# fishaudio/fish-diffusion

Hardware: NVIDIA H100
Metric: mel_frames_per_sec_100step_ddpm (higher is better)
Workload: dtype f32 (3x fp16 split-product wgmma, fp32 accumulate)

## Files before the change

fish_diffusion_b200/csrc/fd_common.cuh:

```cuda
#pragma once
#include <cuda_runtime.h>
#include <cuda_fp16.h>
#include <cuda_bf16.h>
#include <stdint.h>

#define FD_F16 0
#define FD_BF16 1
#define FD_SINGLE 0x10

#define FD_MAX_SEG 16

#define FD_EPI_LINEAR 0
#define FD_EPI_GATE 1
#define FD_EPI_RES_SKIP 2
#define FD_EPI_MAG 3
#define FD_EPI_GATE_BWD 4

#define FD_ACT_NONE 0
#define FD_ACT_RELU 1
#define FD_ACT_LRELU 2
#define FD_ACT_GELU 3

struct FdSeg {
  int src;
// ... 73 lines not shown

__device__ __forceinline__ void fd_split(float v, int prec, uint16_t& hi, uint16_t& lo) {
  if (prec == FD_F16) {
    v = fminf(fmaxf(v, -65504.f), 65504.f);
    __half h = __float2half_rn(v);
    __half l = __float2half_rn(v - __half2float(h));
    hi = __half_as_ushort(h);
    lo = __half_as_ushort(l);
  } else {
    __nv_bfloat16 h = __float2bfloat16_rn(v);
    __nv_bfloat16 l = __float2bfloat16_rn(v - __bfloat162float(h));
    hi = __bfloat16_as_ushort(h);
    lo = __bfloat16_as_ushort(l);
  }
}

__device__ __forceinline__ float fd_h2f(uint16_t u, int prec) {
  if (prec == FD_F16) return __half2float(__ushort_as_half(u));
  return __uint_as_float(((uint32_t)u) << 16);
}

__device__ __forceinline__ float fd_combine(uint16_t hi, uint16_t lo, int prec) {
  return fd_h2f(hi, prec) + fd_h2f(lo, prec);
}

__device__ __forceinline__ void fd_combine2(uint32_t hi2, uint32_t lo2, int prec, float& a, float& b) {
  if (prec == FD_F16) {
    const float2 h = __half22float2(*reinterpret_cast<const __half2*>(&hi2));
    const float2 l = __half22float2(*reinterpret_cast<const __half2*>(&lo2));
    a = h.x + l.x; b = h.y + l.y;
  } else {
    a = __uint_as_float(hi2 << 16) + __uint_as_float(lo2 << 16);
    b = __uint_as_float(hi2 & 0xffff0000u) + __uint_as_float(lo2 & 0xffff0000u);
  }
}

__device__ __forceinline__ float fd_act(float w, float slope) { return fmaf(slope, fminf(w, 0.f), fmaxf(w, 0.f)); }

__device__ __forceinline__ float fd_gelu(float x) { return 0.5f * x * (1.f + erff(x * 0.70710678118654752440f)); }

__device__ __forceinline__ float fd_sigmoid(float x) { return __fdividef(1.f, 1.f + __expf(-x)); }
__device__ __forceinline__ float fd_tanh(float x) {
  float ax = fabsf(x);
  if (ax < 0.04f) { float x2 = x * x; return x * (1.f - x2 * (0.33333333f - 0.13333333f * x2)); }
  float e = __expf(2.f * ax);
  float r = 1.f - __fdividef(2.f, e + 1.f);
  return copysignf(r, x);
}

__device__ __forceinline__ void fd_dgate(float dz, float g, float f, float& dg, float& df) {
  const float sg = fd_sigmoid(g), th = fd_tanh(f);
  dg = dz * th * sg * (1.f - sg);
  df = dz * sg * (1.f - th * th);
}

__device__ __forceinline__ void fd_split2(float a, float b, int prec, uint32_t& hi2, uint32_t& lo2) {
  if (prec == FD_F16) {
    asm("cvt.rn.satfinite.f16x2.f32 %0, %1, %2;" : "=r"(hi2) : "f"(b), "f"(a));
    const float2 hf = __half22float2(*reinterpret_cast<const __half2*>(&hi2));
    asm("cvt.rn.satfinite.f16x2.f32 %0, %1, %2;" : "=r"(lo2) : "f"(b - hf.y), "f"(a - hf.x));
  } else {
    asm("cvt.rn.satfinite.bf16x2.f32 %0, %1, %2;" : "=r"(hi2) : "f"(b), "f"(a));
    const float ha = __uint_as_float(hi2 << 16), hb = __uint_as_float(hi2 & 0xffff0000u);
    asm("cvt.rn.satfinite.bf16x2.f32 %0, %1, %2;" : "=r"(lo2) : "f"(b - hb), "f"(a - ha));
  }
}

template <int V>
__device__ __forceinline__ void fd_store_planes(uint16_t* planes, size_t plane_elems, size_t off,
                                                const float (&y)[V], int prec) {
  uint32_t hi[V / 2], lo[V / 2];
#pragma unroll
  for (int i = 0; i < V / 2; ++i) fd_split2(y[2 * i], y[2 * i + 1], prec, hi[i], lo[i]);
  if (V == 4) {
    *reinterpret_cast<uint2*>(planes + off) = make_uint2(hi[0], hi[1]);
    *reinterpret_cast<uint2*>(planes + plane_elems + off) = make_uint2(lo[0], lo[1]);
  } else {
    *reinterpret_cast<uint4*>(planes + off) = make_uint4(hi[0], hi[1], hi[2 % (V / 2)], hi[3 % (V / 2)]);
    *reinterpret_cast<uint4*>(planes + plane_elems + off) = make_uint4(lo[0], lo[1], lo[2 % (V / 2)], lo[3 % (V / 2)]);
  }
}

template <int V>
__device__ __forceinline__ void fd_load_planes(const uint16_t* planes, size_t plane_elems, size_t off,
                                               float (&y)[V], int prec) {
  uint32_t hi[4], lo[4];
  if (V == 4) {
    const uint2 a = *reinterpret_cast<const uint2*>(planes + off);
    const uint2 b = *reinterpret_cast<const uint2*>(planes + plane_elems + off);
    hi[0] = a.x; hi[1] = a.y; lo[0] = b.x; lo[1] = b.y;
  } else {
    const uint4 a = *reinterpret_cast<const uint4*>(planes + off);
    const uint4 b = *reinterpret_cast<const uint4*>(planes + plane_elems + off);
    hi[0] = a.x; hi[1] = a.y; hi[2] = a.z; hi[3] = a.w; lo[0] = b.x; lo[1] = b.y; lo[2] = b.z; lo[3] = b.w;
  }
#pragma unroll
  for (int i = 0; i < V / 2; ++i) fd_combine2(hi[i], lo[i], prec, y[2 * i], y[2 * i + 1]);
}

__device__ __forceinline__ void fd_load_hi8(const uint16_t* planes, size_t off, float (&y)[8], int prec) {
  const uint4 a = *reinterpret_cast<const uint4*>(planes + off);
  const uint32_t w[4] = {a.x, a.y, a.z, a.w};
#pragma unroll
  for (int i = 0; i < 4; ++i) {
    y[2 * i] = fd_h2f((uint16_t)(w[i] & 0xffff), prec);
    y[2 * i + 1] = fd_h2f((uint16_t)(w[i] >> 16), prec);
  }
}

template <int V>
__device__ __forceinline__ void fd_load_f32(const float* p, float (&y)[V]) {
#pragma unroll
  for (int i = 0; i < V; i += 4) {
    float4 q = *reinterpret_cast<const float4*>(p + i);
    y[i] = q.x; y[i + 1] = q.y; y[i + 2] = q.z; y[i + 3] = q.w;
  }
}
template <int V>
__device__ __forceinline__ void fd_store_f32(float* p, const float (&y)[V]) {
#pragma unroll
  for (int i = 0; i < V; i += 4)
    *reinterpret_cast<float4*>(p + i) = make_float4(y[i], y[i + 1], y[i + 2], y[i + 3]);
}

template <typename I>
struct FdRows {
  I item;
  int t0, dt, nrows;
  __device__ __forceinline__ I row(const FdTapGemm& p, int r) const { return item + (I)min(t0 + r * dt, p.T - 1); }
};

__device__ __forceinline__ int fd_gate_col(const FdTapGemm& p, int c) {
  const int half = p.gate_tile / 2;
  return (c / half) * p.gate_tile + c % half;
}

template <int R, int V, int PREC, typename I>
__device__ __forceinline__ void fd_epi_linear(const FdTapGemm& p, const FdRows<I>& rw, int n, float (&a)[R][V],
                                              const float (&bias)[V]) {
  const int prec = PREC < 0 ? p.prec : PREC;
  const size_t plane = (size_t)p.B * p.T * p.n_total;
  I off[R];
  float pre[R][V];
#pragma unroll
  for (int r = 0; r < R; ++r) {
    off[r] = rw.row(p, r) * (I)p.n_total + (I)n;
#pragma unroll
    for (int i = 0; i < V; ++i) pre[r][i] = 0.f;
  }
  if (p.addend != nullptr) {
#pragma unroll
    for (int r = 0; r < R; ++r) {
      float v[V];
      fd_load_f32<V>(p.addend + off[r], v);
#pragma unroll
      for (int i = 0; i < V; ++i) pre[r][i] += v[i];
    }
  }
  if (p.res_f32 != nullptr) {
#pragma unroll
    for (int r = 0; r < R; ++r) {
      float v[V];
      fd_load_f32<V>(p.res_f32 + off[r], v);
#pragma unroll
      for (int i = 0; i < V; ++i) pre[r][i] += v[i];
    }
  }
  if (p.res_planes != nullptr) {
#pragma unroll
    for (int r = 0; r < R; ++r) {
      float v[V];
      fd_load_planes<V>(p.res_planes, plane, off[r], v, prec);
#pragma unroll
      for (int i = 0; i < V; ++i) pre[r][i] += p.res_scale * v[i];
    }
  }
  uint32_t masked = 0;
  if (p.row_mask != nullptr) {
#pragma unroll
    for (int r = 0; r < R; ++r)
      if (p.row_mask[rw.row(p, r)] != 0) masked |= 1u << r;
  }
#pragma unroll
  for (int r = 0; r < R; ++r)
#pragma unroll
    for (int i = 0; i < V; ++i) a[r][i] = (a[r][i] * p.acc_scale + bias[i] + pre[r][i]) * p.post_scale;
  if (p.out_f32 != nullptr && p.out_accum) {
#pragma unroll
    for (int r = 0; r < R; ++r) {
      float v[V];
      fd_load_f32<V>(p.out_f32 + off[r], v);
#pragma unroll
      for (int i = 0; i < V; ++i) a[r][i] += v[i];
    }
  }
  const float slope = p.act == FD_ACT_NONE ? 1.f : p.act == FD_ACT_RELU ? 0.f : p.act_slope;
#pragma unroll
  for (int r = 0; r < R; ++r) {
    if (r >= rw.nrows) break;
    if ((masked >> r) & 1u) {
#pragma unroll
      for (int i = 0; i < V; ++i) a[r][i] = 0.f;
    }
    if (p.out_f32 != nullptr) fd_store_f32<V>(p.out_f32 + off[r], a[r]);
    if (p.out_planes != nullptr) {
      float v[V];
      if (p.act == FD_ACT_GELU) {
#pragma unroll
        for (int i = 0; i < V; ++i) v[i] = fd_gelu(a[r][i] * p.planes_scale);
      } else {
#pragma unroll
        for (int i = 0; i < V; ++i) v[i] = fd_act(a[r][i] * p.planes_scale, slope);
      }
      fd_store_planes<V>(p.out_planes, plane, off[r], v, prec);
    }
  }
}

template <int R, int V, int PREC, typename I>
__device__ __forceinline__ void fd_epi_res_skip(const FdTapGemm& p, const FdRows<I>& rw, int n, bool is_res,
                                                const float (&a)[R][V], const float (&bias)[V]) {
  const int prec = PREC < 0 ? p.prec : PREC;
  const size_t plane = (size_t)p.B * p.T * p.C;
  const I cn = (I)(is_res ? n : n - p.C);
  I off[R];
#pragma unroll
  for (int r = 0; r < R; ++r) off[r] = rw.row(p, r) * (I)p.C + cn;
  if (is_res) {
    if (p.last_layer) return;
    float x[R][V];
#pragma unroll
    for (int r = 0; r < R; ++r) fd_load_planes<V>(p.x_planes, plane, off[r], x[r], prec);
    uint16_t* const xo = p.x_out_planes != nullptr ? p.x_out_planes : p.x_planes;
#pragma unroll
    for (int r = 0; r < R; ++r) {
      if (r >= rw.nrows) break;
#pragma unroll
      for (int i = 0; i < V; ++i) x[r][i] = (x[r][i] + (a[r][i] * p.acc_scale + bias[i])) * 0.70710678118654752440f;
      fd_store_planes<V>(xo, plane, off[r], x[r], prec);
    }
  } else {
    float sk[R][V];
    if (!p.first_layer) {
#pragma unroll
      for (int r = 0; r < R; ++r) fd_load_f32<V>(p.skip_f32 + off[r], sk[r]);
    }
#pragma unroll
    for (int r = 0; r < R; ++r) {
      if (r >= rw.nrows) break;
      float y[V];
#pragma unroll
      for (int i = 0; i < V; ++i) {
        y[i] = a[r][i] * p.acc_scale + bias[i];
        if (!p.first_layer) y[i] += sk[r][i];
      }
      if (p.last_layer) {
#pragma unroll
        for (int i = 0; i < V; ++i) y[i] *= p.skip_scale;
        fd_store_planes<V>(p.skip_planes, plane, off[r], y, prec);
      } else {
        fd_store_f32<V>(p.skip_f32 + off[r], y);
      }
    }
  }
}

template <int V>
__device__ __forceinline__ void fd_epi_gate(const FdTapGemm& p, int t, float (&g)[V], float (&f)[V], float (&z)[V],
                                            const float (&bias)[2][V], const float (&add)[2][V],
                                            const float (&lo)[2][V], const float (&hi)[2][V]) {
#pragma unroll
  for (int i = 0; i < V; ++i) {
    g[i] = g[i] * p.acc_scale + bias[0][i];
    f[i] = f[i] * p.acc_scale + bias[1][i];
  }
  if (p.addend != nullptr) {
#pragma unroll
    for (int i = 0; i < V; ++i) { g[i] += add[0][i]; f[i] += add[1][i]; }
  }
  if (t < p.dil) {
#pragma unroll
    for (int i = 0; i < V; ++i) { g[i] -= lo[0][i]; f[i] -= lo[1][i]; }
  }
  if (t + p.dil >= p.T) {
#pragma unroll
    for (int i = 0; i < V; ++i) { g[i] -= hi[0][i]; f[i] -= hi[1][i]; }
  }
#pragma unroll
  for (int i = 0; i < V; ++i) z[i] = fd_sigmoid(g[i]) * fd_tanh(f[i]);
}

template <int V>
struct FdColSums {
  float all[2][V], lo[2][V], hi[2][V];
};

template <int R, int V, int PREC, typename I>
__device__ __forceinline__ void fd_epi_gate_bwd(const FdTapGemm& p, const FdRows<I>& rw, int n, const float (&a)[R][V],
                                                FdColSums<V>& s) {
  const int prec = PREC < 0 ? p.prec : PREC;
  const int half = p.gate_tile / 2;
  const I w2 = 2 * (I)p.C, pg = (I)fd_gate_col(p, n);
  const size_t plane = (size_t)p.B * p.T * w2;
  I off[R];
  float g[R][V], f[R][V];
#pragma unroll
  for (int r = 0; r < R; ++r) {
    off[r] = rw.row(p, r) * w2 + pg;
    fd_load_planes<V>(p.y_planes, plane, off[r], g[r], prec);
    fd_load_planes<V>(p.y_planes, plane, off[r] + half, f[r], prec);
  }
  const bool sums = p.cs != nullptr || p.cs_edge != nullptr;
#pragma unroll
  for (int r = 0; r < R; ++r) {
    if (r >= rw.nrows) break;
    float dg[V], df[V];
#pragma unroll
    for (int i = 0; i < V; ++i) fd_dgate(a[r][i] * p.acc_scale, g[r][i], f[r][i], dg[i], df[i]);
    fd_store_planes<V>(p.out_planes, plane, off[r], dg, prec);
    fd_store_planes<V>(p.out_planes, plane, off[r] + half, df, prec);
    if (sums) {
      const int t = rw.t0 + r * rw.dt;
      const bool in_lo = t < p.dil, in_hi = t + p.dil >= p.T;
#pragma unroll
      for (int i = 0; i < V; ++i) {
        s.all[0][i] += dg[i]; s.all[1][i] += df[i];
        if (in_lo) { s.lo[0][i] += dg[i]; s.lo[1][i] += df[i]; }
        if (in_hi) { s.hi[0][i] += dg[i]; s.hi[1][i] += df[i]; }
      }
    }
  }
}

template <int FIRST_XOR, int V>
__device__ __forceinline__ void fd_gate_bwd_colsums(const FdTapGemm& p, FdColSums<V>& s, bool edge_lo, bool edge_hi,
                                                    bool lead, int b, int n) {
  if (p.cs == nullptr && p.cs_edge == nullptr) return;
  auto butterfly = [](float (&x)[2][V], int i) {
#pragma unroll
    for (int h = 0; h < 2; ++h)
#pragma unroll
      for (int o = FIRST_XOR; o < 32; o *= 2) x[h][i] += __shfl_xor_sync(0xffffffffu, x[h][i], o);
  };
#pragma unroll
// ... 73 lines not shown
```

fish_diffusion_b200/csrc/fd_tapgemm_simt.cu:

```cuda
#include "fd_common.cuh"

namespace {

constexpr int BM = 128;
constexpr int BK = 16;
constexpr int APITCH = BM + 4;

template <int RUN, int EPI>
__global__ void __launch_bounds__(256) fd_tapgemm_simt_kernel(const FdTapGemm p) {
  constexpr int BN = 2 * RUN;
  constexpr int TXC = RUN / 4;
  constexpr int TYC = 256 / TXC;
  constexpr int RM = BM / TYC;
  constexpr int BPITCH = BN + 4;

  __shared__ float As[BK][APITCH];
  __shared__ float Bs[BK][BPITCH];

  const int tid = threadIdx.x;
  const int tx = tid % TXC, ty = tid / TXC;
  const int tiles_t = (p.T + BM - 1) / BM;
  const int m_tile = blockIdx.x;
  const int b = m_tile / tiles_t;
  const int t0 = (m_tile % tiles_t) * BM;
// ... 51 lines not shown
#pragma unroll
          for (int i = 0; i < 8; ++i) v[i] = 0.f;
        }
#pragma unroll
        for (int i = 0; i < 8; ++i) Bs[kh * 8 + i][nl] = v[i];
      }
      __syncthreads();
#pragma unroll
      for (int k = 0; k < BK; ++k) {
        float a[RM], bv[8];
#pragma unroll
        for (int r = 0; r < RM; ++r) a[r] = As[k][ty * RM + r];
        float4 b0 = *reinterpret_cast<const float4*>(&Bs[k][tx * 4]);
        float4 b1 = *reinterpret_cast<const float4*>(&Bs[k][RUN + tx * 4]);
        bv[0] = b0.x; bv[1] = b0.y; bv[2] = b0.z; bv[3] = b0.w;
        bv[4] = b1.x; bv[5] = b1.y; bv[6] = b1.z; bv[7] = b1.w;
#pragma unroll
        for (int r = 0; r < RM; ++r)
#pragma unroll
          for (int c = 0; c < 8; ++c) acc[r][c] = fmaf(a[r], bv[c], acc[r][c]);
      }
      __syncthreads();
    }
    koff += sg.k_len;
  }

  const int tr = t0 + ty * RM, nrows = max(0, min(RM, p.T - tr));
  if constexpr (EPI == FD_EPI_GATE || EPI == FD_EPI_MAG) {
    const int zc = j * RUN + tx * 4, n_g = run0 + tx * 4, n_f = run1 + tx * 4;
    if (n_g >= p.n_total) return;
    const size_t zplane = (size_t)p.B * p.T * p.C, yplane = (size_t)p.B * p.T * p.n_total;
#pragma unroll
    for (int r = 0; r < RM; ++r) {
      if (r >= nrows) break;
      const int t = tr + r;
      float g[4] = {acc[r][0], acc[r][1], acc[r][2], acc[r][3]};
      float f[4] = {acc[r][4], acc[r][5], acc[r][6], acc[r][7]};
      if constexpr (EPI == FD_EPI_MAG) {
        fd_epi_mag<4>(p, b, t, zc, g, f);
      } else {
        const size_t row = (size_t)b * p.T + t, bo = (size_t)b * p.gbias_bstride;
        float add[2][4], bias[2][4], lo[2][4], hi[2][4], z[4];
        if (p.addend != nullptr) {
          fd_load_f32<4>(p.addend + row * p.n_total + n_g, add[0]);
          fd_load_f32<4>(p.addend + row * p.n_total + n_f, add[1]);
        }
#pragma unroll
        for (int i = 0; i < 4; ++i) {
          bias[0][i] = p.gbias_full[bo + n_g + i]; bias[1][i] = p.gbias_full[bo + n_f + i];
          lo[0][i] = p.gbias_lo[bo + n_g + i]; lo[1][i] = p.gbias_lo[bo + n_f + i];
          hi[0][i] = p.gbias_hi[bo + n_g + i]; hi[1][i] = p.gbias_hi[bo + n_f + i];
        }
        fd_epi_gate<4>(p, t, g, f, z, bias, add, lo, hi);
        if (p.y_planes != nullptr) {
          fd_store_planes<4>(p.y_planes, yplane, row * p.n_total + n_g, g, p.prec);
          fd_store_planes<4>(p.y_planes, yplane, row * p.n_total + n_f, f, p.prec);
        }
        fd_store_planes<4>(p.out_planes, zplane, row * p.C + zc, z, p.prec);
      }
    }
  } else {
#pragma unroll
    for (int h = 0; h < 2; ++h) {
      const int n = (h == 0 ? run0 : run1) + tx * 4;
      if constexpr (EPI == FD_EPI_GATE_BWD) {
        FdColSums<4> s{};
#pragma unroll
        for (int r = 0; r < RM; ++r) {
          if (r >= nrows || n >= p.n_total) break;
          float a[1][4] = {{acc[r][4 * h], acc[r][4 * h + 1], acc[r][4 * h + 2], acc[r][4 * h + 3]}};
          fd_epi_gate_bwd<1, 4, -1>(p, FdRows<size_t>{(size_t)b * p.T, tr + r, 1, 1}, n, a, s);
        }
        fd_gate_bwd_colsums<TXC>(p, s, t0 < p.dil, t0 + BM + p.dil > p.T, tid % 32 < TXC && n < p.n_total, b, n);
      } else {
        if (n >= p.n_total) continue;
#pragma unroll
        for (int r = 0; r < RM; ++r) {
          if (r >= nrows) break;
          float bias[4];
#pragma unroll
          for (int i = 0; i < 4; ++i) bias[i] = p.bias != nullptr ? p.bias[(size_t)b * p.bias_bstride + n + i] : 0.f;
          float a[1][4] = {{acc[r][4 * h], acc[r][4 * h + 1], acc[r][4 * h + 2], acc[r][4 * h + 3]}};
          const FdRows<size_t> row{(size_t)b * p.T, tr + r, 1, 1};
          if constexpr (EPI == FD_EPI_LINEAR) fd_epi_linear<1, 4, -1>(p, row, n, a, bias);
          else fd_epi_res_skip<1, 4, -1>(p, row, n, n < p.C, a, bias);
        }
      }
    }
  }
}

template <int RUN>
int launch_run(const FdTapGemm& p, cudaStream_t stream) {
  const int tiles_t = (p.T + BM - 1) / BM;
  dim3 grid(p.B * tiles_t, 1, 1), block(256);
  if (p.epi == FD_EPI_GATE) {
    grid.y = (p.n_total / 2 + RUN - 1) / RUN;
    fd_tapgemm_simt_kernel<RUN, FD_EPI_GATE><<<grid, block, 0, stream>>>(p);
  } else if (p.epi == FD_EPI_MAG) {
    grid.y = (p.n_total / 2 + RUN - 1) / RUN;
    fd_tapgemm_simt_kernel<RUN, FD_EPI_MAG><<<grid, block, 0, stream>>>(p);
  } else if (p.epi == FD_EPI_RES_SKIP) {
    grid.y = (p.n_total + 2 * RUN - 1) / (2 * RUN);
    fd_tapgemm_simt_kernel<RUN, FD_EPI_RES_SKIP><<<grid, block, 0, stream>>>(p);
  } else if (p.epi == FD_EPI_GATE_BWD) {
    grid.y = (p.n_total + 2 * RUN - 1) / (2 * RUN);
    fd_tapgemm_simt_kernel<RUN, FD_EPI_GATE_BWD><<<grid, block, 0, stream>>>(p);
  } else {
    grid.y = (p.n_total + 2 * RUN - 1) / (2 * RUN);
    fd_tapgemm_simt_kernel<RUN, FD_EPI_LINEAR><<<grid, block, 0, stream>>>(p);
  }
  FD_CHECK_CUDA(cudaGetLastError());
  return 0;
}

constexpr int WG_R = 64, WG_C = 64, WG_T = 16;

__global__ void __launch_bounds__(256) fd_wgrad_simt_kernel(const FdWgradK p, const uint16_t* row0,
                                                            const uint16_t* row1, const uint16_t* col0,
                                                            const uint16_t* col1, int prec, int single) {
  static_assert(WG_R == WG_C, "rows and columns share the staging code");
  __shared__ __align__(16) float Rs[WG_T][WG_R + 4];
  __shared__ __align__(16) float Cs[WG_T][WG_C + 4];
  const int tid = threadIdx.x;
  const int s = blockIdx.z, r0 = blockIdx.y * WG_R, c0 = blockIdx.x * WG_C;

  const bool is_col = tid >= 128;
  const int grp = tid % 8, tl = (tid % 128) / 8;
  const int i = (is_col ? c0 : r0) + grp * 8;
  const uint16_t* src = nullptr;
  int C = 0, ch = 0, shift = 0;
  if (!is_col) {
    for (int g = 0; g < p.num_row_seg; ++g)
      if (i >= p.row_start[g] && i < p.row_start[g] + p.row_width[g]) {
        src = p.row_src[g] == 0 ? row0 : row1;
        C = p.row_C[p.row_src[g]]; ch = p.row_coff[g] + (i - p.row_start[g]);
      }
  } else {
    for (int g = 0; g < p.num_col_seg; ++g)
      if (i >= p.col_start[g] && i < p.col_start[g] + p.col_width[g]) {
        src = p.col_src[g] == 0 ? col0 : col1;
        C = p.col_C[p.col_src[g]]; ch = p.col_coff[g] + (i - p.col_start[g]); shift = p.col_shift[g];
      }
  }
  const size_t plane = (size_t)p.B * p.T * C;
  float* const dst = is_col ? &Cs[tl][grp * 8] : &Rs[tl][grp * 8];

  const int tx = tid % 16, ty = tid / 16;
  float acc[4][4];
#pragma unroll
  for (int r = 0; r < 4; ++r)
#pragma unroll
    for (int c = 0; c < 4; ++c) acc[r][c] = 0.f;

  const int b_end = min(p.B, (s + 1) * p.items_per_split);
  for (int b = s * p.items_per_split; b < b_end; ++b) {
    for (int t0 = 0; t0 < p.T; t0 += WG_T) {
      const int t = t0 + tl, ts = t + shift;
      float v[8];
      if (src != nullptr && t < p.T && ts >= 0 && ts < p.T) {
        const size_t off = ((size_t)b * p.T + ts) * C + ch;
        if (single) fd_load_hi8(src, off, v, prec);
        else fd_load_planes<8>(src, plane, off, v, prec);
      } else {
#pragma unroll
        for (int k = 0; k < 8; ++k) v[k] = 0.f;
      }
      *reinterpret_cast<float4*>(dst) = make_float4(v[0], v[1], v[2], v[3]);
// ... 62 lines not shown
```

fish_diffusion_b200/csrc/fd_tapgemm_tc.cu:

```cuda
#include <cuda.h>
#include "fd_common.cuh"
#include "fd_host.h"
#include "fd_tc_ptx.cuh"

namespace {

constexpr int BLOCK_M = 128;

template <int BLOCK_N, int BLOCK_K, int EPI, int NPL>
struct Cfg {
  static constexpr bool PP = EPI == FD_EPI_GATE || EPI == FD_EPI_RES_SKIP;
  static constexpr int ROWS = PP ? 64 : BLOCK_M;
  static constexpr int A_BYTES = ROWS * BLOCK_K * 2;
  static constexpr int W_BYTES = BLOCK_N * BLOCK_K * 2;
  static constexpr int GROUP = BLOCK_K >= 64 || PP ? 1 : 64 / BLOCK_K;
  static constexpr int SUB_BYTES = NPL * (A_BYTES + W_BYTES);
  static constexpr int STAGE_BYTES = GROUP * SUB_BYTES;
  static constexpr int TX_BYTES = SUB_BYTES;
  static constexpr int SWIZZLE_BYTES = BLOCK_K * 2;
  static constexpr uint32_t SWIZZLE_MODE = swizzle_mode_for(SWIZZLE_BYTES);
  static constexpr uint32_t SBO = 8 * SWIZZLE_BYTES;
  static constexpr int BIAS_FLOATS = (EPI == FD_EPI_GATE ? 3 : 1) * BLOCK_N;
  static constexpr int BIAS_TOTAL = (PP ? 2 : 1) * BIAS_FLOATS;
  static constexpr int NUM_STAGES = fd_tc_frame_stages(STAGE_BYTES, BIAS_TOTAL);
  static constexpr int SMEM_BYTES = fd_tc_frame_bytes(NUM_STAGES, STAGE_BYTES, BIAS_TOTAL);
  static_assert(NUM_STAGES >= 2, "pipeline needs at least two stages");
  static_assert(SMEM_BYTES <= FD_TC_SMEM_BUDGET, "shared memory");
};

template <int BLOCK_N, int EPI>
__device__ __forceinline__ void stage_bias(const FdTapGemm& p, int b, int n0, float* bias_s, int i0, int step) {
  if (EPI == FD_EPI_GATE) {
    const size_t bo = (size_t)b * p.gbias_bstride + n0;
    for (int i = i0; i < BLOCK_N; i += step) {
      bias_s[i] = p.gbias_full[bo + i];
      bias_s[BLOCK_N + i] = p.gbias_lo[bo + i];
      bias_s[2 * BLOCK_N + i] = p.gbias_hi[bo + i];
    }
  } else {
    for (int i = i0; i < BLOCK_N; i += step)
      bias_s[i] = p.bias ? p.bias[(size_t)b * p.bias_bstride + n0 + i] : 0.f;
  }
}
template <int EPI>
__device__ __forceinline__ long long bias_key(const FdTapGemm& p, int b, int n0) {
  return EPI == FD_EPI_GATE ? (long long)b * p.gbias_bstride + n0 : (long long)b * p.bias_bstride + n0;
}

template <int BLOCK_N, int EPI, int PREC>
__device__ __forceinline__ void tile_epilogue(const FdTapGemm& p, const float* acc, int b, int n_tile, int rw0,
                                              const float* bias_s, uint32_t my_scratch, int lane) {
  const int n0 = n_tile * BLOCK_N;
  if constexpr (EPI == FD_EPI_GATE || EPI == FD_EPI_MAG) {
    constexpr int HALF = BLOCK_N / 2;
    const uint32_t sb = smem_u32(bias_s);
    const int r = lane >> 1, sub = lane & 1;
    const int t = rw0 + r;
    const bool valid = t < p.T;
    const bool e_lo = t < p.dil, e_hi = t + p.dil >= p.T;
    const bool edge_any = __any_sync(0xffffffffu, valid && (e_lo || e_hi));
    const size_t zplane = (size_t)p.B * p.T * p.C, zrow = ((size_t)b * p.T + t) * p.C + (size_t)n_tile * HALF;
    const size_t yplane = (size_t)p.B * p.T * p.n_total, yrow = ((size_t)b * p.T + t) * p.n_total;
#pragma unroll
    for (int c = 0; c < HALF; c += 16) {
      frag_to_scratch<16>(my_scratch, acc, c, 0, lane);
      frag_to_scratch<16>(my_scratch, acc, HALF + c, 16, lane);
      __syncwarp();
      float g[8], f[8];
      {
        const float4 g0 = scratch_ld4(my_scratch, r, 2 * sub), g1 = scratch_ld4(my_scratch, r, 2 * sub + 1);
        const float4 f0 = scratch_ld4(my_scratch, r, 4 + 2 * sub), f1 = scratch_ld4(my_scratch, r, 5 + 2 * sub);
        g[0] = g0.x; g[1] = g0.y; g[2] = g0.z; g[3] = g0.w; g[4] = g1.x; g[5] = g1.y; g[6] = g1.z; g[7] = g1.w;
        f[0] = f0.x; f[1] = f0.y; f[2] = f0.z; f[3] = f0.w; f[4] = f1.x; f[5] = f1.y; f[6] = f1.z; f[7] = f1.w;
      }
      __syncwarp();
      const int cc = c + 8 * sub;
      if (valid) {
        if (EPI == FD_EPI_MAG) {
          fd_epi_mag<8, PREC>(p, b, t, n_tile * HALF + cc, g, f);
        } else {
          float add[2][8], bias[2][8], lo[2][8], hi[2][8], z[8];
          if (p.addend != nullptr) {
#pragma unroll
            for (int h = 0; h < 2; ++h) ldcs_f32(p.addend + yrow + n0 + h * HALF + cc, add[h]);
          }
#pragma unroll
          for (int h = 0; h < 2; ++h) lds_f32(sb + 4u * (h * HALF + cc), bias[h]);
          if (edge_any) {
#pragma unroll
            for (int h = 0; h < 2; ++h)
              if (e_lo) lds_f32(sb + 4u * (BLOCK_N + h * HALF + cc), lo[h]);
#pragma unroll
            for (int h = 0; h < 2; ++h)
              if (e_hi) lds_f32(sb + 4u * (2 * BLOCK_N + h * HALF + cc), hi[h]);
          }
          fd_epi_gate<8>(p, t, g, f, z, bias, add, lo, hi);
          if (p.y_planes != nullptr) {
            const int ng = p.gate_tile == BLOCK_N ? n0 + cc : fd_gate_col(p, n_tile * HALF + cc);
            fd_store_planes<8>(p.y_planes, yplane, yrow + ng, g, PREC);
            fd_store_planes<8>(p.y_planes, yplane, yrow + ng + p.gate_tile / 2, f, PREC);
          }
          fd_store_planes<8>(p.out_planes, zplane, zrow + cc, z, PREC);
        }
      }
    }
  } else if constexpr (BLOCK_N >= 64) {
    const uint32_t bias_addr = smem_u32(bias_s);
    const int j4 = (lane & 7) * 4, rsub = lane >> 3;
    const int rbase = rw0 + rsub;
    const FdRows<uint32_t> rows{(uint32_t)b * (uint32_t)p.T, rbase, 4,
                                rbase < p.T ? min(4, (p.T - rbase + 3) / 4) : 0};
#pragma unroll
    for (int c = 0; c < BLOCK_N; c += 32) {
      const int col = c + j4;
      const int n = n0 + col;
      frag_to_scratch<32>(my_scratch, acc, c, 0, lane);
      __syncwarp();
      float a[4][4];
#pragma unroll
      for (int r = 0; r < 4; ++r) {
        const float4 x = scratch_ld4(my_scratch, 4 * r + rsub, lane & 7);
        a[r][0] = x.x; a[r][1] = x.y; a[r][2] = x.z; a[r][3] = x.w;
      }
      __syncwarp();
      if constexpr (EPI == FD_EPI_GATE_BWD) {
        FdColSums<4> s{};
        fd_epi_gate_bwd<4, 4, PREC>(p, rows, n, a, s);
        fd_gate_bwd_colsums<8>(p, s, rw0 < p.dil, rw0 + 16 + p.dil > p.T, rsub == 0, b, n);
      } else {
        float bias[4];
        lds_f32(bias_addr + 4u * col, bias);
        if constexpr (EPI == FD_EPI_RES_SKIP) fd_epi_res_skip<4, 4, PREC>(p, rows, n, n0 < p.C, a, bias);
        else fd_epi_linear<4, 4, PREC>(p, rows, n, a, bias);
      }
    }
  } else {
    static_assert(EPI == FD_EPI_LINEAR, "narrow tiles: LINEAR only");
    constexpr int PER = BLOCK_N / 2;
    frag_to_scratch<BLOCK_N>(my_scratch, acc, 0, 0, lane);
    __syncwarp();
    const int r = lane >> 1, sub = lane & 1;
    float v[PER];
#pragma unroll
    for (int q4 = 0; q4 < PER / 4; ++q4) {
      const float4 x = scratch_ld4(my_scratch, r, sub * (PER / 4) + q4);
      v[4 * q4] = x.x; v[4 * q4 + 1] = x.y; v[4 * q4 + 2] = x.z; v[4 * q4 + 3] = x.w;
    }
    __syncwarp();
    const int t = rw0 + r;
    const FdRows<uint32_t> row{(uint32_t)b * (uint32_t)p.T, t, 1, t < p.T ? 1 : 0};
#pragma unroll
    for (int h = 0; h < PER / 8; ++h) {
      const int cc = sub * PER + h * 8;
      float a[1][8], bias[8];
#pragma unroll
      for (int i = 0; i < 8; ++i) a[0][i] = v[h * 8 + i];
      lds_f32(smem_u32(bias_s) + 4u * cc, bias);
      fd_epi_linear<1, 8, PREC>(p, row, n0 + cc, a, bias);
    }
  }
}

template <int BLOCK_N, int BLOCK_K, int EPI, int PREC, int NPL>
__global__ void __launch_bounds__(FD_TC_THREADS, 1)
fd_tapgemm_tc_kernel(const __grid_constant__ CUtensorMap tm_src0, const __grid_constant__ CUtensorMap tm_src1,
                     const __grid_constant__ CUtensorMap tm_w, const FdTapGemm p) {
  using C = Cfg<BLOCK_N, BLOCK_K, EPI, NPL>;
  static_assert(!C::PP, "GATE / RES_SKIP run the ping-pong schedule");
  using MMA = Wgmma<BLOCK_N, PREC>;
  extern __shared__ uint8_t smem_raw[];
  const TcFrame f = tc_frame(smem_raw, C::NUM_STAGES, C::STAGE_BYTES, C::BIAS_TOTAL);
  Ring ring{f.full, f.empty, C::NUM_STAGES};

  const int warp = threadIdx.x / 32;
  const int lane = threadIdx.x % 32;

  const int tiles_t = (p.T + BLOCK_M - 1) / BLOCK_M;
  const int num_m_tiles = p.B * tiles_t;
  const int num_n_tiles = p.n_total / BLOCK_N;
  const int num_tiles = num_m_tiles * num_n_tiles;
  int total_k_blocks = 0;
  for (int sI = 0; sI < p.num_seg; ++sI) total_k_blocks += p.seg[sI].k_len / BLOCK_K;

  tc_prologue<false>(f, C::NUM_STAGES, FD_TC_CONSUMER_THREADS / 32, &tm_src0, &tm_src1, &tm_w);

  if (warp >= FD_TC_PRODUCER_WARP) {
    producer_regs();
    if (warp == FD_TC_PRODUCER_WARP && lane == 0) {
      for (int tile = blockIdx.x; tile < num_tiles; tile += gridDim.x) {
        const int m_tile = tile / num_n_tiles;
        const int n_tile = (tile % num_n_tiles + m_tile) % num_n_tiles;
        const int b = m_tile / tiles_t, t0 = (m_tile % tiles_t) * BLOCK_M;
        const int n0 = n_tile * BLOCK_N;
        SegCursor sc;
        for (int kb = 0; kb < total_k_blocks; kb += C::GROUP) {
          const int nb = min(C::GROUP, total_k_blocks - kb);
          ring.wait_empty();
          uint8_t* st = f.ring + ring.stage * C::STAGE_BYTES;
          mbar_expect_tx(ring.full_bar(), nb * C::TX_BYTES);
          for (int g = 0; g < nb; ++g) {
            const FdSeg sg = p.seg[sc.s];
            const CUtensorMap* tm = sg.src == 0 ? &tm_src0 : &tm_src1;
            uint8_t* sub = st + g * C::SUB_BYTES;
            tma_load_4d(sub, tm, ring.full_bar(), sg.c_off + sc.k0, t0 + sg.shift, b, 0);
            const int kw = sc.koff + sc.k0 + p.w_kshift;
            tma_load_3d(sub + NPL * C::A_BYTES, &tm_w, ring.full_bar(), kw, n0, 0);
            sc.next(BLOCK_K, sg.k_len);
          }
          ring.next();
        }
      }
    }
    return;
  }

  consumer_regs();
  const int wg = warp / 4;
  const int wq = warp % 4;
  const uint32_t my_scratch = smem_u32(f.scratch) + warp * FD_TC_SCRATCH_WARP_BYTES;
  float* bias_s = f.bias;
  float acc[BLOCK_N / 2];
  long long staged_key = -1;
  for (int tile = blockIdx.x; tile < num_tiles; tile += gridDim.x) {
    const int m_tile = tile / num_n_tiles;
    const int n_tile = (tile % num_n_tiles + m_tile) % num_n_tiles;
    const int b = m_tile / tiles_t, t0 = (m_tile % tiles_t) * BLOCK_M;
    const int n0 = n_tile * BLOCK_N;

    if (EPI == FD_EPI_LINEAR && bias_key<EPI>(p, b, n0) != staged_key) {
      staged_key = bias_key<EPI>(p, b, n0);
      named_bar_sync<1, FD_TC_CONSUMER_THREADS>();
      stage_bias<BLOCK_N, EPI>(p, b, n0, bias_s, threadIdx.x, FD_TC_CONSUMER_THREADS);
      named_bar_sync<1, FD_TC_CONSUMER_THREADS>();
    }

    ring_mainloop(acc, ring, total_k_blocks, C::GROUP, lane, [&](int stage, int nb) {
      for (int g = 0; g < nb; ++g) {
        const uint32_t st = smem_u32(f.ring + stage * C::STAGE_BYTES + g * C::SUB_BYTES);
        const uint32_t wg_a = wg * 64 * C::SWIZZLE_BYTES;
        const uint64_t a_hi = make_smem_desc(st + wg_a, 16, C::SBO, C::SWIZZLE_MODE);
        const uint64_t a_lo = make_smem_desc(st + C::A_BYTES + wg_a, 16, C::SBO, C::SWIZZLE_MODE);
        const uint64_t w_hi = make_smem_desc(st + NPL * C::A_BYTES, 16, C::SBO, C::SWIZZLE_MODE);
        const uint64_t w_lo = make_smem_desc(st + NPL * C::A_BYTES + C::W_BYTES, 16, C::SBO, C::SWIZZLE_MODE);
        split_mma<MMA, NPL, BLOCK_K / 16, 32>(acc, a_hi, a_lo, w_hi, w_lo);
      }
    });

    tile_epilogue<BLOCK_N, EPI, PREC>(p, acc, b, n_tile, t0 + wg * 64 + wq * 16, bias_s, my_scratch, lane);
  }
}

template <int BLOCK_N, int BLOCK_K, int EPI, int PREC, int NPL>
__global__ void __launch_bounds__(FD_TC_THREADS, 1)
fd_tapgemm_pp_kernel(const __grid_constant__ CUtensorMap tm_src0, const __grid_constant__ CUtensorMap tm_src1,
                     const __grid_constant__ CUtensorMap tm_w, const FdTapGemm p) {
  using C = Cfg<BLOCK_N, BLOCK_K, EPI, NPL>;
  static_assert(C::PP && C::GROUP == 1, "ping-pong schedule: GATE / RES_SKIP, one k-block per stage");
  using MMA = Wgmma<BLOCK_N, PREC>;
  extern __shared__ uint8_t smem_raw[];
  const TcFrame f = tc_frame(smem_raw, C::NUM_STAGES, C::STAGE_BYTES, C::BIAS_TOTAL);

  const int warp = threadIdx.x / 32;
  const int lane = threadIdx.x % 32;
  const int rank = (int)cluster_ctarank();
  const int pair = blockIdx.x / 2, num_pairs = gridDim.x / 2;

  const int tiles_t = (p.T + 63) / 64;
  const int num_m_tiles = p.B * tiles_t;
  const int num_n_tiles = p.n_total / BLOCK_N;
  const int num_units = (num_m_tiles + 1) / 2 * num_n_tiles;
  int total_k_blocks = 0;
  for (int sI = 0; sI < p.num_seg; ++sI) total_k_blocks += p.seg[sI].k_len / BLOCK_K;

  tc_prologue<true>(f, C::NUM_STAGES, 2 * 4, &tm_src0, &tm_src1, &tm_w);

  if (warp >= FD_TC_PRODUCER_WARP) {
    producer_regs();
    if (warp == FD_TC_PRODUCER_WARP && lane == 0) {
      Ring ring{f.full, f.empty, C::NUM_STAGES};
      for (int u = pair; u < num_units; u += num_pairs) {
        const int m_pair = u / num_n_tiles;
        const int n_tile = (u % num_n_tiles + m_pair) % num_n_tiles;
        const int m_tile = min(2 * m_pair + rank, num_m_tiles - 1);
        const int b = m_tile / tiles_t, t0 = (m_tile % tiles_t) * 64;
        const int n0 = n_tile * BLOCK_N;
        SegCursor sc;
#pragma unroll 1
        for (int kb = 0; kb < total_k_blocks; ++kb) {
          ring.wait_empty();
          uint8_t* st = f.ring + ring.stage * C::STAGE_BYTES;
          mbar_expect_tx(ring.full_bar(), C::TX_BYTES);
          const FdSeg sg = p.seg[sc.s];
          tma_load_4d(st, sg.src == 0 ? &tm_src0 : &tm_src1, ring.full_bar(), sg.c_off + sc.k0, t0 + sg.shift, b, 0);
          tma_load_3d_multicast(st + NPL * C::A_BYTES + rank * (NPL * C::W_BYTES / 2), &tm_w, ring.full_bar(),
                                sc.koff + sc.k0 + p.w_kshift, n0 + (NPL == 1 ? rank * (BLOCK_N / 2) : 0),
                                NPL == 2 ? rank : 0, 0x3);
          sc.next(BLOCK_K, sg.k_len);
          ring.next();
        }
      }
    }
  } else {
    consumer_regs();
    const int wg = warp / 4;
    const int wq = warp % 4;
    const uint32_t my_scratch = smem_u32(f.scratch) + warp * FD_TC_SCRATCH_WARP_BYTES;
    float* my_bias = f.bias + wg * C::BIAS_FLOATS;
    float acc[BLOCK_N / 2];
    PingPong turn(f.full, f.empty, C::NUM_STAGES, total_k_blocks, wg);
    long long staged_key = -1;
    for (int u = pair + wg * num_pairs; u < num_units; u += 2 * num_pairs) {
      const int m_pair = u / num_n_tiles;
      const int n_tile = (u % num_n_tiles + m_pair) % num_n_tiles;
      const int m_tile = 2 * m_pair + rank;
      const bool valid = m_tile < num_m_tiles;
      const int b = m_tile / tiles_t, t0 = (m_tile % tiles_t) * 64;
      const int n0 = n_tile * BLOCK_N;

      if (valid && bias_key<EPI>(p, b, n0) != staged_key) {
        staged_key = bias_key<EPI>(p, b, n0);
        wg == 0 ? named_bar_sync<3, 128>() : named_bar_sync<4, 128>();
        stage_bias<BLOCK_N, EPI>(p, b, n0, my_bias, threadIdx.x % 128, 128);
        wg == 0 ? named_bar_sync<3, 128>() : named_bar_sync<4, 128>();
      }

      turn.mainloop(acc, u == pair, u + num_pairs < num_units, lane, [&](int stage) {
        const uint32_t st = smem_u32(f.ring + stage * C::STAGE_BYTES);
        const uint64_t a_hi = make_smem_desc(st, 16, C::SBO, C::SWIZZLE_MODE);
        const uint64_t a_lo = make_smem_desc(st + C::A_BYTES, 16, C::SBO, C::SWIZZLE_MODE);
        const uint64_t w_hi = make_smem_desc(st + NPL * C::A_BYTES, 16, C::SBO, C::SWIZZLE_MODE);
        const uint64_t w_lo = make_smem_desc(st + NPL * C::A_BYTES + C::W_BYTES, 16, C::SBO, C::SWIZZLE_MODE);
        split_mma<MMA, NPL, BLOCK_K / 16, 32>(acc, a_hi, a_lo, w_hi, w_lo);
      });

      if (valid) tile_epilogue<BLOCK_N, EPI, PREC>(p, acc, b, n_tile, t0 + wq * 16, my_bias, my_scratch, lane);
    }
  }
  __syncwarp();
  cluster_sync();
}

template <int BLOCK_T>
struct GateTCfg {
  static constexpr int BLOCK_K = 32;
  static constexpr int ROW_BYTES = BLOCK_K * 2;
  static constexpr int ACT_ROWS = BLOCK_T + 16;
  static constexpr int MAX_DIL = (ACT_ROWS - BLOCK_T) / 2;
  static constexpr int ACT_PLANE = ACT_ROWS * ROW_BYTES;
  static constexpr int W_PLANE = 64 * ROW_BYTES;
  static constexpr int W_OFF = 2 * ACT_PLANE;
  static constexpr int STAGE_BYTES = W_OFF + 3 * 2 * W_PLANE;
  static constexpr uint32_t SWIZZLE_MODE = swizzle_mode_for(ROW_BYTES);
  static constexpr uint32_t SBO = 8 * ROW_BYTES;
  static constexpr int NUM_STAGES = fd_tc_frame_stages(STAGE_BYTES, 0);
  static constexpr int SMEM_BYTES = fd_tc_frame_bytes(NUM_STAGES, STAGE_BYTES, 0);
  static_assert(ACT_ROWS <= 256, "one TMA box per plane");
  static_assert(ACT_PLANE % 512 == 0 && STAGE_BYTES % 1024 == 0, "planes start on 64 B swizzle atoms");
  static_assert(NUM_STAGES >= 3, "ring depth");
  static_assert(SMEM_BYTES <= FD_TC_SMEM_BUDGET, "shared memory");
};

template <int BLOCK_T, int PREC>
__device__ __forceinline__ void gate_t_epilogue(const FdTapGemm& p, const float* acc, int b, int t0, int ch,
                                                uint32_t my_scratch, int lane) {
  const int half = p.gate_tile / 2;
  const int e = lane >> 2, q4 = lane & 3;
  const int n_g = fd_gate_col(p, ch) + e, n_f = n_g + half;
  const size_t bo = (size_t)b * p.gbias_bstride;
  const float bias[2][1] = {{p.gbias_full[bo + n_g]}, {p.gbias_full[bo + n_f]}};
  const float lo[2][1] = {{p.gbias_lo[bo + n_g]}, {p.gbias_lo[bo + n_f]}};
  const float hi[2][1] = {{p.gbias_hi[bo + n_g]}, {p.gbias_hi[bo + n_f]}};
  const size_t row0 = (size_t)b * p.T;
  const size_t zplane = (size_t)p.B * p.T * p.C;
  constexpr int NG = BLOCK_T / 8;
  auto load_addend = [&](int c0, float (&a)[16]) {
#pragma unroll
    for (int i = 0; i < 16; ++i) a[i] = 0.f;
    if (p.addend == nullptr) return;
#pragma unroll
    for (int ci = 0; ci < 4; ++ci) {
      if (c0 + ci < NG) {
#pragma unroll
        for (int s = 0; s < 2; ++s) {
          const int t = min(t0 + 8 * (c0 + ci) + 2 * q4 + s, p.T - 1);
          const float* ad = p.addend + (row0 + t) * p.n_total;
          a[4 * ci + 2 * s] = __ldcs(ad + n_g);
          a[4 * ci + 2 * s + 1] = __ldcs(ad + n_f);
        }
      }
    }
  };
  float a_next[16];
  load_addend(0, a_next);
#pragma unroll
  for (int c0 = 0; c0 < NG; c0 += 4) {
    float a_cur[16];
#pragma unroll
    for (int i = 0; i < 16; ++i) a_cur[i] = a_next[i];
    if (c0 + 4 < NG) load_addend(c0 + 4, a_next);
#pragma unroll
    for (int ci = 0; ci < 4; ++ci) {
      if (c0 + ci < NG) {
#pragma unroll
        for (int s = 0; s < 2; ++s) {
          const int tl = 8 * ci + 2 * q4 + s;
          const int t = t0 + 8 * c0 + tl;
          float g[1] = {acc[4 * (c0 + ci) + s]}, f[1] = {acc[4 * (c0 + ci) + 2 + s]}, z[1];
          const float add[2][1] = {{a_cur[4 * ci + 2 * s]}, {a_cur[4 * ci + 2 * s + 1]}};
          fd_epi_gate<1>(p, t, g, f, z, bias, add, lo, hi);
          sts32(my_scratch + 4u * (tl * 8 + (((e >> 2) ^ ((tl >> 2) & 1)) << 2) + (e & 3)), z[0]);
        }
      }
    }
    __syncwarp();
    const int t = t0 + 8 * c0 + lane;
    if (lane < 8 * min(4, NG - c0) && t < p.T) {
      const uint32_t sw = (uint32_t)((lane >> 2) & 1);
      const float4 z0 = lds128(my_scratch + 4u * (lane * 8 + (sw << 2)));
// ... 256 lines not shown
```

Measured before the change: 22750.

## Prefetch residual/skip epilogue operands before mainloop and software-pipeline epilogue loads

Splits the residual/skip epilogue into a load phase and an apply phase. In the ping-pong tensor-core kernel, the first few column chunks of x planes and skip f32 values are fetched into registers before the MMA mainloop. Later chunks are prefetched DEPTH chunks ahead inside the epilogue, so global-load latency overlaps with compute. The cost is extra register pressure from holding up to DEPTH×16 words per thread across the mainloop, which could hurt occupancy or cause spills.

After: 23000, median of 6. 1.01x the previous value.

```diff
diff --git a/fish_diffusion_b200/csrc/fd_common.cuh b/fish_diffusion_b200/csrc/fd_common.cuh
--- a/fish_diffusion_b200/csrc/fd_common.cuh
+++ b/fish_diffusion_b200/csrc/fd_common.cuh
@@ -179,20 +179,30 @@
 }
 
 template <int V>
-__device__ __forceinline__ void fd_load_planes(const uint16_t* planes, size_t plane_elems, size_t off,
-                                               float (&y)[V], int prec) {
-  uint32_t hi[4], lo[4];
-  if (V == 4) {
+__device__ __forceinline__ void fd_load_plane_words(const uint16_t* planes, size_t plane_elems, size_t off,
+                                                    uint32_t (&w)[V]) {
+  if constexpr (V == 4) {
     const uint2 a = *reinterpret_cast<const uint2*>(planes + off);
     const uint2 b = *reinterpret_cast<const uint2*>(planes + plane_elems + off);
-    hi[0] = a.x; hi[1] = a.y; lo[0] = b.x; lo[1] = b.y;
+    w[0] = a.x; w[1] = a.y; w[2] = b.x; w[3] = b.y;
   } else {
     const uint4 a = *reinterpret_cast<const uint4*>(planes + off);
     const uint4 b = *reinterpret_cast<const uint4*>(planes + plane_elems + off);
-    hi[0] = a.x; hi[1] = a.y; hi[2] = a.z; hi[3] = a.w; lo[0] = b.x; lo[1] = b.y; lo[2] = b.z; lo[3] = b.w;
-  }
-#pragma unroll
-  for (int i = 0; i < V / 2; ++i) fd_combine2(hi[i], lo[i], prec, y[2 * i], y[2 * i + 1]);
+    w[0] = a.x; w[1] = a.y; w[2] = a.z; w[3] = a.w; w[4] = b.x; w[5] = b.y; w[6] = b.z; w[7] = b.w;
+  }
+}
+template <int V>
+__device__ __forceinline__ void fd_combine_words(const uint32_t (&w)[V], float (&y)[V], int prec) {
+#pragma unroll
+  for (int i = 0; i < V / 2; ++i) fd_combine2(w[i], w[V / 2 + i], prec, y[2 * i], y[2 * i + 1]);
+}
+
+template <int V>
+__device__ __forceinline__ void fd_load_planes(const uint16_t* planes, size_t plane_elems, size_t off,
+                                               float (&y)[V], int prec) {
+  uint32_t w[V];
+  fd_load_plane_words<V>(planes, plane_elems, off, w);
+  fd_combine_words<V>(w, y, prec);
 }
 
 __device__ __forceinline__ void fd_load_hi8(const uint16_t* planes, size_t off, float (&y)[8], int prec) {
@@ -314,49 +324,65 @@
   }
 }
 
+template <typename I>
+__device__ __forceinline__ I fd_res_skip_off(const FdTapGemm& p, const FdRows<I>& rw, int n, bool is_res, int r) {
+  return rw.row(p, r) * (I)p.C + (I)(is_res ? n : n - p.C);
+}
+
+template <int R, int V, typename I>
+__device__ __forceinline__ void fd_epi_res_skip_load(const FdTapGemm& p, const FdRows<I>& rw, int n, bool is_res,
+                                                     uint32_t (&w)[R][V]) {
+  if (is_res ? p.last_layer : p.first_layer) return;
+  const size_t plane = (size_t)p.B * p.T * p.C;
+#pragma unroll
+  for (int r = 0; r < R; ++r) {
+    const I off = fd_res_skip_off(p, rw, n, is_res, r);
+    if (is_res) {
+      fd_load_plane_words<V>(p.x_planes, plane, off, w[r]);
+    } else {
+      float sk[V];
+      fd_load_f32<V>(p.skip_f32 + off, sk);
+#pragma unroll
+      for (int i = 0; i < V; ++i) w[r][i] = __float_as_uint(sk[i]);
+    }
+  }
+}
+
 template <int R, int V, int PREC, typename I>
-__device__ __forceinline__ void fd_epi_res_skip(const FdTapGemm& p, const FdRows<I>& rw, int n, bool is_res,
-                                                const float (&a)[R][V], const float (&bias)[V]) {
+__device__ __forceinline__ void fd_epi_res_skip_apply(const FdTapGemm& p, const FdRows<I>& rw, int n, bool is_res,
+                                                      const float (&a)[R][V], const float (&bias)[V],
+                                                      const uint32_t (&w)[R][V]) {
   const int prec = PREC < 0 ? p.prec : PREC;
   const size_t plane = (size_t)p.B * p.T * p.C;
-  const I cn = (I)(is_res ? n : n - p.C);
-  I off[R];
-#pragma unroll
-  for (int r = 0; r < R; ++r) off[r] = rw.row(p, r) * (I)p.C + cn;
   if (is_res) {
     if (p.last_layer) return;
-    float x[R][V];
-#pragma unroll
-    for (int r = 0; r < R; ++r) fd_load_planes<V>(p.x_planes, plane, off[r], x[r], prec);
     uint16_t* const xo = p.x_out_planes != nullptr ? p.x_out_planes : p.x_planes;
 #pragma unroll
     for (int r = 0; r < R; ++r) {
       if (r >= rw.nrows) break;
-#pragma unroll
-      for (int i = 0; i < V; ++i) x[r][i] = (x[r][i] + (a[r][i] * p.acc_scale + bias[i])) * 0.70710678118654752440f;
-      fd_store_planes<V>(xo, plane, off[r], x[r], prec);
+      float x[V];
+      fd_combine_words<V>(w[r], x, prec);
+#pragma unroll
+      for (int i = 0; i < V; ++i) x[i] = (x[i] + (a[r][i] * p.acc_scale + bias[i])) * 0.70710678118654752440f;
+      fd_store_planes<V>(xo, plane, fd_res_skip_off(p, rw, n, is_res, r), x, prec);
     }
   } else {
-    float sk[R][V];
-    if (!p.first_layer) {
-#pragma unroll
-      for (int r = 0; r < R; ++r) fd_load_f32<V>(p.skip_f32 + off[r], sk[r]);
-    }
 #pragma unroll
     for (int r = 0; r < R; ++r) {
       if (r >= rw.nrows) break;
+      const I off = fd_res_skip_off(p, rw, n, is_res, r);
       float y[V];
 #pragma unroll
       for (int i = 0; i < V; ++i) {
         y[i] = a[r][i] * p.acc_scale + bias[i];
-        if (!p.first_layer) y[i] += sk[r][i];
+        if (!p.first_layer) y[i] += __uint_as_float(w[r][i]);
       }
       if (p.last_layer) {
 #pragma unroll
         for (int i = 0; i < V; ++i) y[i] *= p.skip_scale;
-        fd_store_planes<V>(p.skip_planes, plane, off[r], y, prec);
+        fd_store_planes<V>(p.skip_planes, plane, off, y, prec);
       } else {
-        fd_store_f32<V>(p.skip_f32 + off[r], y);
+        fd_store_f32<V>(p.skip_f32 + off, y);
       }
     }
   }
diff --git a/fish_diffusion_b200/csrc/fd_tapgemm_simt.cu b/fish_diffusion_b200/csrc/fd_tapgemm_simt.cu
--- a/fish_diffusion_b200/csrc/fd_tapgemm_simt.cu
+++ b/fish_diffusion_b200/csrc/fd_tapgemm_simt.cu
@@ -157,8 +157,13 @@
           for (int i = 0; i < 4; ++i) bias[i] = p.bias != nullptr ? p.bias[(size_t)b * p.bias_bstride + n + i] : 0.f;
           float a[1][4] = {{acc[r][4 * h], acc[r][4 * h + 1], acc[r][4 * h + 2], acc[r][4 * h + 3]}};
           const FdRows<size_t> row{(size_t)b * p.T, tr + r, 1, 1};
-          if constexpr (EPI == FD_EPI_LINEAR) fd_epi_linear<1, 4, -1>(p, row, n, a, bias);
-          else fd_epi_res_skip<1, 4, -1>(p, row, n, n < p.C, a, bias);
+          if constexpr (EPI == FD_EPI_LINEAR) {
+            fd_epi_linear<1, 4, -1>(p, row, n, a, bias);
+          } else {
+            uint32_t w[1][4];
+            fd_epi_res_skip_load<1, 4>(p, row, n, n < p.C, w);
+            fd_epi_res_skip_apply<1, 4, -1>(p, row, n, n < p.C, a, bias, w);
+          }
         }
       }
     }
diff --git a/fish_diffusion_b200/csrc/fd_tapgemm_tc.cu b/fish_diffusion_b200/csrc/fd_tapgemm_tc.cu
--- a/fish_diffusion_b200/csrc/fd_tapgemm_tc.cu
+++ b/fish_diffusion_b200/csrc/fd_tapgemm_tc.cu
@@ -47,9 +47,34 @@
   return EPI == FD_EPI_GATE ? (long long)b * p.gbias_bstride + n0 : (long long)b * p.bias_bstride + n0;
 }
 
+__device__ __forceinline__ FdRows<uint32_t> coalesced_rows(const FdTapGemm& p, int b, int rw0, int lane) {
+  const int rbase = rw0 + (lane >> 3);
+  return {(uint32_t)b * (uint32_t)p.T, rbase, 4, rbase < p.T ? min(4, (p.T - rbase + 3) / 4) : 0};
+}
+
+template <int BLOCK_N, int EPI>
+struct EpiPrefetch {
+  __device__ __forceinline__ void start(const FdTapGemm&, int, int, int, int) {}
+};
+template <int BLOCK_N>
+struct EpiPrefetch<BLOCK_N, FD_EPI_RES_SKIP> {
+  static constexpr int CHUNKS = BLOCK_N / 32;
+  static constexpr int DEPTH = CHUNKS < 8 ? CHUNKS : 3;
+  uint32_t w[DEPTH][4][4];
+  __device__ __forceinline__ void load(const FdTapGemm& p, const FdRows<uint32_t>& rows, int n0, int c, int lane) {
+    fd_epi_res_skip_load<4, 4>(p, rows, n0 + 32 * c + 4 * (lane & 7), n0 < p.C, w[c % DEPTH]);
+  }
+  __device__ __forceinline__ void start(const FdTapGemm& p, int b, int n0, int rw0, int lane) {
+    const FdRows<uint32_t> rows = coalesced_rows(p, b, rw0, lane);
+#pragma unroll
+    for (int c = 0; c < DEPTH; ++c) load(p, rows, n0, c, lane);
+  }
+};
+
 template <int BLOCK_N, int EPI, int PREC>
 __device__ __forceinline__ void tile_epilogue(const FdTapGemm& p, const float* acc, int b, int n_tile, int rw0,
-                                              const float* bias_s, uint32_t my_scratch, int lane) {
+                                              const float* bias_s, uint32_t my_scratch, int lane,
+                                              EpiPrefetch<BLOCK_N, EPI>& pf) {
   const int n0 = n_tile * BLOCK_N;
   if constexpr (EPI == FD_EPI_GATE || EPI == FD_EPI_MAG) {
     constexpr int HALF = BLOCK_N / 2;
@@ -107,9 +132,7 @@
   } else if constexpr (BLOCK_N >= 64) {
     const uint32_t bias_addr = smem_u32(bias_s);
     const int j4 = (lane & 7) * 4, rsub = lane >> 3;
-    const int rbase = rw0 + rsub;
-    const FdRows<uint32_t> rows{(uint32_t)b * (uint32_t)p.T, rbase, 4,
-                                rbase < p.T ? min(4, (p.T - rbase + 3) / 4) : 0};
+    const FdRows<uint32_t> rows = coalesced_rows(p, b, rw0, lane);
 #pragma unroll
     for (int c = 0; c < BLOCK_N; c += 32) {
       const int col = c + j4;
@@ -130,8 +153,14 @@
       } else {
         float bias[4];
         lds_f32(bias_addr + 4u * col, bias);
-        if constexpr (EPI == FD_EPI_RES_SKIP) fd_epi_res_skip<4, 4, PREC>(p, rows, n, n0 < p.C, a, bias);
-        else fd_epi_linear<4, 4, PREC>(p, rows, n, a, bias);
+        if constexpr (EPI == FD_EPI_RES_SKIP) {
+          constexpr int DEPTH = EpiPrefetch<BLOCK_N, EPI>::DEPTH;
+          const int k = c / 32;
+          fd_epi_res_skip_apply<4, 4, PREC>(p, rows, n, n0 < p.C, a, bias, pf.w[k % DEPTH]);
+          if (k + DEPTH < BLOCK_N / 32) pf.load(p, rows, n0, k + DEPTH, lane);
+        } else {
+          fd_epi_linear<4, 4, PREC>(p, rows, n, a, bias);
+        }
       }
     }
   } else {
@@ -220,6 +249,7 @@
   const uint32_t my_scratch = smem_u32(f.scratch) + warp * FD_TC_SCRATCH_WARP_BYTES;
   float* bias_s = f.bias;
   float acc[BLOCK_N / 2];
+  EpiPrefetch<BLOCK_N, EPI> pf;
   long long staged_key = -1;
   for (int tile = blockIdx.x; tile < num_tiles; tile += gridDim.x) {
     const int m_tile = tile / num_n_tiles;
@@ -246,7 +276,7 @@
       }
     });
 
-    tile_epilogue<BLOCK_N, EPI, PREC>(p, acc, b, n_tile, t0 + wg * 64 + wq * 16, bias_s, my_scratch, lane);
+    tile_epilogue<BLOCK_N, EPI, PREC>(p, acc, b, n_tile, t0 + wg * 64 + wq * 16, bias_s, my_scratch, lane, pf);
   }
 }
 
@@ -307,6 +337,7 @@
     const uint32_t my_scratch = smem_u32(f.scratch) + warp * FD_TC_SCRATCH_WARP_BYTES;
     float* my_bias = f.bias + wg * C::BIAS_FLOATS;
     float acc[BLOCK_N / 2];
+    EpiPrefetch<BLOCK_N, EPI> pf;
     PingPong turn(f.full, f.empty, C::NUM_STAGES, total_k_blocks, wg);
     long long staged_key = -1;
     for (int u = pair + wg * num_pairs; u < num_units; u += 2 * num_pairs) {
@@ -324,6 +355,8 @@
         wg == 0 ? named_bar_sync<3, 128>() : named_bar_sync<4, 128>();
       }
 
+      if (valid) pf.start(p, b, n0, t0 + wq * 16, lane);
+
       turn.mainloop(acc, u == pair, u + num_pairs < num_units, lane, [&](int stage) {
         const uint32_t st = smem_u32(f.ring + stage * C::STAGE_BYTES);
         const uint64_t a_hi = make_smem_desc(st, 16, C::SBO, C::SWIZZLE_MODE);
@@ -333,7 +366,7 @@
         split_mma<MMA, NPL, BLOCK_K / 16, 32>(acc, a_hi, a_lo, w_hi, w_lo);
       });
 
-      if (valid) tile_epilogue<BLOCK_N, EPI, PREC>(p, acc, b, n_tile, t0 + wq * 16, my_bias, my_scratch, lane);
+      if (valid) tile_epilogue<BLOCK_N, EPI, PREC>(p, acc, b, n_tile, t0 + wq * 16, my_bias, my_scratch, lane, pf);
     }
   }
   __syncwarp();
```
